# bertoldi-collab/DifFlexMM

Hardware: AMD Instinct MI355X
Metric: timesteps*rigid-units/s (forward + adjoint) (higher is better)
Workload: dtype f64

## Files before the change

difflexmm_amd/csrc/dfx_persist.h:

```cpp
#pragma once
#include "dfx_persist_api.h"

namespace {
using namespace dfx_persist;

typedef unsigned p_u4 __attribute__((ext_vector_type(4)));

__device__ __forceinline__ bool is_poison(double x) { return (unsigned)__double2hiint(x) == kPoisonWord; }

__device__ __forceinline__ void ring_load(const double* place, u32 byte_off, double (&r)[4]) {
  p_u4 c0, c1;
  asm volatile("global_load_dwordx4 %0, %2, %3 sc1\n\tglobal_load_dwordx4 %1, %2, %3 offset:16 sc1\n\ts_waitcnt vmcnt(0)"
               : "=&v"(c0), "=&v"(c1) : "v"(byte_off), "s"(place) : "memory");
  r[0] = __hiloint2double(c0.y, c0.x); r[1] = __hiloint2double(c0.w, c0.z);
  r[2] = __hiloint2double(c1.y, c1.x); r[3] = __hiloint2double(c1.w, c1.z);
}
__device__ __forceinline__ void ring_store(double* place, u32 byte_off, double a, double b) {
  p_u4 x;
  x.x = __double2loint(a); x.y = __double2hiint(a); x.z = __double2loint(b); x.w = __double2hiint(b);
  asm volatile("global_store_dwordx4 %0, %1, %2 sc1\n\ts_nop 1" ::"v"(byte_off), "v"(x), "s"(place) : "memory");
}
__device__ __forceinline__ void ring_poison(double* place, u32 byte_off) {
  p_u4 x; x.x = x.y = x.z = x.w = kPoisonWord;
  asm volatile("global_store_dwordx4 %0, %1, %2 sc1\n\ts_nop 1" ::"v"(byte_off), "v"(x), "s"(place) : "memory");
}

__global__ __launch_bounds__(kThreads) void k_ring_poison(double* ring, int batch, int n_blocks, int m0, int width , int places) {
  const int m = blockIdx.y + m0;
  const int tid = blockIdx.x * kThreads + threadIdx.x;
  if (tid >= n_blocks * width) return;
  const unsigned long long p = ~0ull;
  for (int pl = 0; pl < places; ++pl)
    reinterpret_cast<unsigned long long*>(ring)[((size_t)pl * batch + m) * ((size_t)n_blocks * width) + tid] = p;
}

struct LigRes {
  double rox, roy, rpx, rpy, lx, ly, l0, il0, ks, ksh, kr, sgn;
  double am, ac, kc, phi1, phi2, kap_safe, phi_min;
  int info, pslot;
};
template <int CONTACT, class Ctx >
__device__ __forceinline__ void load_lig_res(const Ctx& c, const MemberBases& B, int slot, LigRes& g) {
  g.info = ldg<int>(c.slot_info, (u32)slot * 4);
  g.pslot = g.info < 0 ? slot : (g.info >> 1);
  g.sgn = (g.info & 1) ? 1.0 : -1.0;
  const double2 ro = ldg<double2>(B.p_r, (u32)slot * 16), rp = ldg<double2>(B.p_r, (u32)g.pslot * 16);
  g.rox = ro.x; g.roy = ro.y; g.rpx = rp.x; g.rpy = rp.y;
  if (c.l_dict_on) {
    const u32 li = (u32)ldg<uint8_t>(B.p_lidx, (u32)slot);
    const double2 lv = ldg<double2>(B.l_dict, li * 32), ln = ldg<double2>(B.l_dict, li * 32 + 16);
    g.lx = lv.x; g.ly = lv.y; g.l0 = ln.x; g.il0 = ln.y;
  } else {
    const double2 lv = ldg<double2>(B.p_l, (u32)slot * 16);
    g.lx = lv.x; g.ly = lv.y;
    g.l0 = g.info < 0 ? 1.0 : sqrt(lv.x * lv.x + lv.y * lv.y);
    g.il0 = 1.0 / g.l0;
  }
  if (c.k_uniform) { g.ks = B.cst[3]; g.ksh = B.cst[4]; g.kr = B.cst[5]; }
  else { g.ks = ldg<double>(B.p_k, (u32)slot * 32); g.ksh = ldg<double>(B.p_k, (u32)slot * 32 + 8); g.kr = ldg<double>(B.p_k, (u32)slot * 32 + 16); }
  g.am = g.ac = g.kc = g.phi1 = g.phi2 = g.kap_safe = g.phi_min = 0.0;
  if (CONTACT == 1) {
    g.am = B.cst[0]; g.ac = B.cst[1]; g.kc = B.cst[2]; g.kap_safe = B.cst[9]; g.phi_min = B.cst[10];
    const double2 ph = ldg<double2>(B.p_phi, (u32)slot * 16);
    g.phi1 = ph.x; g.phi2 = ph.y;
  }
}
__device__ __forceinline__ int fresh_v(int x) { asm volatile("" : "+v"(x)); return x; }
__device__ __forceinline__ MemberBases persist_bases(const PersistCtx& c, u32 um) {
  MemberBases B{};
  const u32 ps = um * (u32)c.n_slots;
  B.p_r = c.p_r + (size_t)(ps * 2); B.p_phi = c.p_phi + (size_t)(ps * 2); B.p_l = c.p_l + (size_t)(ps * 2); B.p_k = c.p_k + (size_t)(ps * 4);
  B.cst = c.cst + (size_t)(um * 16); B.l_dict = c.l_dict + (size_t)(um * 1024); B.p_lidx = c.p_lidx + (size_t)ps;
  return B;
}
__device__ __forceinline__ bool ring_wait(const double* place, u32 byte_off, double (&r)[4], int t_ord, int* give_up, int limit) {
  for (int spins = 0;;) {
    ring_load(place, byte_off, r);
    const bool ok = !(is_poison(r[0]) || is_poison(r[1]) || is_poison(r[2]) || is_poison(r[3]));
    if (__all(ok)) return true;
    if (++spins > limit) { *give_up = 1 + t_ord; return false; }
    __builtin_amdgcn_s_sleep(1);
  }
}

#ifdef DFX_PERSIST_TIMING
__device__ __forceinline__ unsigned long long tick() {
  unsigned long long t;
  asm volatile("s_waitcnt vmcnt(0) lgkmcnt(0)\n\ts_memtime %0\n\ts_waitcnt lgkmcnt(0)" : "=s"(t)::"memory");
  return t;
}
#if DFX_PERSIST_TIMING == 2
#define DFX_TICK(k) if ((k) < 4) { unsigned long long t_; asm volatile("s_memtime %0\n\ts_waitcnt lgkmcnt(0)" : "=s"(t_)::"memory"); acc_t[k] += (unsigned)(t_ - t_prev); t_prev = t_; }
#else
#define DFX_TICK(k) { const unsigned long long t_ = tick(); acc_t[k] += (unsigned)(t_ - t_prev); t_prev = t_; }
#endif
#else
#define DFX_TICK(k)
#endif

__device__ __forceinline__ bool persist_wave(const PersistArgs& pa, int& ml, int& w) {
  const int wv = (int)(threadIdx.x >> 6);
  if (pa.xcd_wg > 0) {
    const int xcd = (int)(blockIdx.x & 7), pos = (int)(blockIdx.x >> 3);
    const int mi = pos / pa.xcd_wg, j = pos - mi * pa.xcd_wg;
    ml = __builtin_amdgcn_readfirstlane(mi * 8 + xcd);
    w = __builtin_amdgcn_readfirstlane(j * (kPersistThreads / 64) + wv);
    return ml < pa.nm && w < pa.waves_per_member;
  }
  const int wave = __builtin_amdgcn_readfirstlane((int)(blockIdx.x * (kPersistThreads / 64)) + wv);
  if (wave >= pa.waves_per_member * pa.nm) return false;
  ml = wave / pa.waves_per_member;
  w = wave - ml * pa.waves_per_member;
  return true;
}

template <int NPB>
__device__ __forceinline__ LanePos wave_lane_pos(int w, int n_blocks) {
  LanePos p;
  const int gtid = w * 64 + (int)(threadIdx.x & 63);
  if (NPB == 4) { p.slot = gtid; p.b = gtid >> 2; p.k = gtid & 3; p.valid = p.b < n_blocks; return p; }
  const int j = gtid & 15;
  const int tri = min((j * 11) >> 5, 4);
  p.k = j - 3 * tri;
  p.b = (gtid >> 4) * 5 + tri;
  p.valid = p.b < n_blocks;
  p.slot = p.b * 4 + p.k;
  return p;
}

#ifndef DFX_PERSIST_OCC
#define DFX_PERSIST_OCC
#endif
template <int MODEL, int CONTACT, int NPB>
__global__ __launch_bounds__(kPersistThreads) DFX_PERSIST_OCC void k_fwd_persist(PersistCtx c, PersistFwdTab pc, PersistArgs pa) {
  int ml, w;
  if (!persist_wave(pa, ml, w)) return;
  const LanePos lp = wave_lane_pos<NPB>(w, c.n_blocks);
  if (!lp.valid) return;
  const int slot = lp.slot, b = lp.b, k = lp.k, kd = k < 3 ? k : 2;
  const u32 um = (u32)ml;
  const u32 nd = (u32)c.n_blocks * 3;
  const int s = c.s;
  const Seg sg = *c.cur;
  const MemberBases B = persist_bases(c, um);
  LigRes g;
  load_lig_res<CONTACT>(c, B, slot, g);
  const int info = g.info, pslot = g.pslot;
  const int dof = b * 3 + kd;
  const u32 o_dof = (u32)dof * 8, o_rec = ((u32)b * kPos + kd) * 8, o_chunk = ((u32)b * kPos + 2 * (k & 1)) * 8;
  const double damp = c.damping_uniform ? B.cst[6 + kd] : ldg<double>(c.damping + (size_t)(um * nd), o_dof);
  const double invm = ldg<double>(c.inv_m + (size_t)(um * nd), o_dof);
  const int sidx = ldg<int>(c.block_special, (u32)b * 4);
  const bool constrained = k < 3 && sidx >= 0 && ((c.special[sidx >= 0 ? sidx : 0].con_mask >> k) & 1);
  double tf_coef[DFX_MAX_FNS];
#pragma unroll
  for (int f = 0; f < DFX_MAX_FNS; ++f)
    tf_coef[f] = (k < 3 && sidx >= 0 && f < c.n_fns) ? (constrained ? c.special[sidx].con_coef[k][f] : c.special[sidx].load_coef[k][f]) : 0.0;
  const bool recs = c.rps > 1;
  const long long n0 = sg.base_step;
  const size_t blk = (size_t)((u32)c.n_blocks * (u32)kStep);
  const size_t rec_step = (size_t)(u32)c.batch * blk;
// ... 2 lines not shown
  double* const VELm = c.VEL + (size_t)(um * (u32)c.nbuf * nd);
  double qn, vn;
  BlockRec<double> o;
  {
    const double* P0 = recs ? traj_m + (size_t)((u32)n0 * (u32)c.rps) * rec_step : POSm;
    const double* V0 = recs ? P0 + (size_t)((u32)c.n_blocks * (u32)kPos) : VELm;
    const double2 a0 = ldg<double2>(P0, (u32)b * kPos * 8), a1 = ldg<double2>(P0, (u32)b * kPos * 8 + 16);
    o.x = a0.x; o.y = a0.y; o.th = a1.x; o.sh = a1.y;
    qn = ldg<double>(P0, o_rec);
    vn = ldg<double>(V0, o_dof);
  }
  double al[kPersistStages];
#pragma unroll
  for (int l = 0; l < kPersistStages; ++l) al[l] = 0.0;
  const size_t ring_stride = (size_t)((u32)c.batch * (u32)c.n_blocks * (u32)kPos);
  const u32 r_own = (um * (u32)c.n_blocks + (u32)b) * (kPos * 8) + 16u * (u32)(k & 1);
  const u32 r_par = (um * (u32)c.n_blocks + (u32)(pslot >> 2)) * (kPos * 8);
  if (k < 2) ring_store(pa.ring, r_own, k == 0 ? o.x : o.th, k == 0 ? o.y : o.sh);
  const int total = pa.n_steps * s;
  int t_ord = 0;
  double v_i = vn;
  const int keep = recs ? 2 : (c.traj ? 1 : 0);
  double* tr = keep ? traj_m + ((size_t)((u32)n0 * (u32)c.rps) + 1) * rec_step : nullptr;
  const size_t rec_adv = recs ? rec_step : 0, rec_gap = recs ? (size_t)(u32)(c.rps - s) * rec_step : (keep ? rec_step : 0);
  const u32 o_vrec = (u32)c.n_blocks * (kPos * 8) + o_dof;
  const double* ft = c.fn_tab ? c.fn_tab + ((size_t)um * kMaxGraphSteps * kFnRows) * (DFX_MAX_FNS * kFnEntry) : nullptr;
  const int ft_row = c.fn_tab ? DFX_MAX_FNS * kFnEntry : 0;
  const u32 z_row = constrained ? (u32)(DFX_MAX_FNS * kFnEntry * 8) : 0u;
  double* Am = c.AD ? c.AD + (size_t)um * c.ad_stride + (size_t)n0 * ((u32)(s - 1) * nd) : nullptr;
  const double* place = pa.ring;
#ifdef DFX_PERSIST_TIMING
  unsigned acc_t[6] = {0, 0, 0, 0, 0, 0};
  unsigned long long t_prev = tick();
  const unsigned long long t_first = t_prev, w_first = wall_clock64();
#endif
  for (int j = 0; j < pa.n_steps; ++j) {
    const long long n = n0 + j;
    double h = sg.h;
    if (c.t_steps) { const double* ts = c.t_steps + (size_t)um * (size_t)c.ts_stride; h = ts[n + 1] - ts[n]; }
#pragma unroll 1
    for (int i = 0; i < s; ++i) {
      {
        const double* row = pc.row[i];
        double cv[kPersistStages - 1], cq[kPersistStages - 1];
#pragma unroll
        for (int l = 0; l < kPersistStages - 1; ++l) { cv[l] = row[l]; cq[l] = row[kPersistStages - 1 + l]; }
        const double cv_i = row[10], cq_i = row[11], c_next = row[12];
        o.ch = half_cos(o.th, o.sh);
        double sv = 0.0, sq = 0.0, fload = 0.0;
#pragma unroll
        for (int l = 0; l < kPersistStages - 1; ++l) {
          sv += cv[l] * al[l];
          sq += cq[l] * al[l];
        }
        double tv0[DFX_MAX_FNS], tv1[DFX_MAX_FNS];
#pragma unroll
        for (int f = 0; f < DFX_MAX_FNS; ++f) { tv0[f] = 0.0; tv1[f] = 0.0; }
        if (k < 3 && sidx >= 0) {
          const u32 z = lane_zero() + z_row;
#pragma unroll
          for (int f = 0; f < DFX_MAX_FNS; ++f)
            if (f < c.n_fns) { tv0[f] = fn_tab_get(ft, f, 0, z); if (constrained) tv1[f] = fn_tab_get(ft, f, 1, z); }
        }
        DFX_TICK(0)
        double pr[4];
        if (!ring_wait(place, r_par, pr, t_ord, pa.give_up, pa.spin_limit)) return;
        DFX_TICK(1)
        if (k < 2 && t_ord + kPAhead <= total) ring_poison(pa.ring + (size_t)(((u32)t_ord + kPAhead) & (kPRing - 1)) * ring_stride, r_own);
        BlockRec<double> p;
        p.x = pr[0]; p.y = pr[1]; p.th = pr[2]; p.sh = pr[3];
        p.ch = half_cos(p.th, p.sh);
        double q_pre = 0.0, v_pre = 0.0;
#pragma unroll
        for (int f = 0; f < DFX_MAX_FNS; ++f) {
          if (constrained) { q_pre += tf_coef[f] * tv0[f]; v_pre += tf_coef[f] * tv1[f]; }
          else fload += tf_coef[f] * tv0[f];
        }
        double fx = 0.0, fy = 0.0, fth = 0.0;
        if (info >= 0) {
          BondGrad<double> bg;
          bond_grad<MODEL, double>(o, p, g.rox, g.roy, g.rpx, g.rpy, g.lx, g.ly, g.l0, g.il0, g.ks, g.ksh, g.kr, g.sgn, bg);
          fx = bg.fx; fy = bg.fy; fth = bg.fth;
          if (CONTACT == 1) {
            const bool far = !(fabs(o.th - p.th) <= g.kap_safe);
            ContactGrad<double> cg;
            contact_grad<double>(g.sgn * (o.th - p.th), far ? g.phi1 : g.phi_min, far ? g.phi2 : g.phi_min, g.am, g.ac, g.kc, cg);
            fth += g.sgn * cg.dkap;
          }
        }
        DFX_TICK(2)
        const double dE = blk_reduce3<NPB>(fx, fy, fth, k);
        double qnext = 0.0, vnext = 0.0;
        if (k < 3) {
          const double a = constrained ? 0.0 : (fload - dE - damp * v_i) * invm;
          if (Am && i < s - 1) stg<double>(Am, o_dof, a);
          sv += cv_i * a;
          sq += cq_i * a;
#pragma unroll
          for (int l = 0; l < kPersistStages; ++l) al[l] = l == i ? a : al[l];
          qnext = qn + h * (c_next * vn + h * sq);
          vnext = vn + h * sv;
          if (constrained) { qnext = q_pre; vnext = v_pre; }
        }
        DFX_TICK(3)
        const double y1 = blk_bcast<NPB, 1>(qnext, k), th2 = blk_bcast<NPB, 2>(qnext, k), x0 = blk_bcast<NPB, 0>(qnext, k);
        double sn, cs;
        fast_sincos(0.5 * th2, &sn, &cs);
        o.x = x0; o.y = y1; o.th = th2; o.sh = sn;
        ++t_ord;
        place = pa.ring + (size_t)((u32)t_ord & (kPRing - 1)) * ring_stride;
        DFX_TICK(4)
        const bool last = i == s - 1;
        if (k < 2) ring_store(const_cast<double*>(place), r_own, k == 0 ? x0 : th2, k == 0 ? y1 : sn);
        if (k < 3) {
          const double2 chunk = k == 0 ? make_double2(x0, y1) : make_double2(th2, sn);
          if (keep > (last ? 0 : 1)) {
            if (k < 2) stg<double2>(tr, o_chunk, chunk);
            stg<double>(tr, o_vrec, vnext);
          }
          if (last && keep < 2 && j == pa.n_steps - 1) {
            if (k < 2) stg<double2>(POSm, o_chunk, chunk);
            stg<double>(VELm, o_dof, vnext);
          }
        }
        v_i = vnext;
        if (last) { qn = qnext; vn = vnext; }
        DFX_TICK(5)
        tr += rec_adv;
        ft += ft_row;
        if (Am && i < s - 1) Am += nd;
      }
    }
    tr += rec_gap;
    ft += (kFnRows - s) * ft_row;
  }
#ifdef DFX_PERSIST_TIMING
  if (pa.dbg && (threadIdx.x & 63) == 0) {
    unsigned* d = pa.dbg + (size_t)(blockIdx.x * 4 + (threadIdx.x >> 6)) * 8;
    for (int q = 0; q < 6; ++q) d[q] = acc_t[q];
    d[6] = (unsigned)(tick() - t_first); d[7] = (unsigned)total;
  }
  if (blockIdx.x == 0 && threadIdx.x == 0) {
    for (int q = 0; q < 6; ++q) pa.give_up[1 + q] = (int)acc_t[q];
    pa.give_up[7] = (int)(tick() - t_first);
    pa.give_up[8] = (int)(wall_clock64() - w_first);
    pa.give_up[9] = total;
  }
#endif
}



template <int MODEL, int CONTACT, int NPB, int DENSE>
__device__ __forceinline__ void adj_persist_body(const PersistCtx& c, const PersistAdjTab& pc, const PersistArgs& pa, const DenseCtx& dn) {
  int ml, w;
  if (!persist_wave(pa, ml, w)) return;
  const LanePos lp = wave_lane_pos<NPB>(w, c.n_blocks);
  if (!lp.valid) return;
  const int slot = lp.slot, b = lp.b, k = lp.k, kd = k < 3 ? k : 2;
  const u32 um = (u32)ml;
  const u32 nd = (u32)c.n_blocks * 3, nd6 = (u32)c.n_blocks * 6;
  const int s = c.s;
  const Seg sg = *c.cur;
  long long n_m = 0;
  int j_top = pa.n_steps - 1;
  if constexpr (DENSE) {
    n_m = dn.n_acc[c.m0 + ml];
    if (n_m - sg.base_step < (long long)j_top) j_top = (int)(n_m - sg.base_step);
    if (j_top < 0) return;
  }
  const MemberBases B = persist_bases(c, um);
  LigRes g;
  load_lig_res<CONTACT>(c, B, slot, g);
  const int info = g.info, pslot = g.pslot;
  const int dof = b * 3 + kd;
  const u32 o_dof = (u32)dof * 8, o_b6 = ((u32)b * 6 + 2 * kd) * 8;
  const double damp = c.damping_uniform ? B.cst[6 + kd] : ldg<double>(c.damping + (size_t)(um * nd), o_dof);
  const double invm = ldg<double>(c.inv_m + (size_t)(um * nd), o_dof);
  const int sidx = ldg<int>(c.block_special, (u32)b * 4);
  const bool constrained = k < 3 && sidx >= 0 && ((c.special[sidx >= 0 ? sidx : 0].con_mask >> k) & 1);
  double tf_coef[DFX_MAX_FNS];
#pragma unroll
  for (int f = 0; f < DFX_MAX_FNS; ++f)
    tf_coef[f] = (k < 3 && sidx >= 0 && f < c.n_fns) ? (constrained ? c.special[sidx].con_coef[k][f] : c.special[sidx].load_coef[k][f]) : 0.0;
  double* LAMm = c.LAM + (size_t)(um * nd6);
  const u32 ms = um * (u32)c.n_slots;
  double* grm = c.g_r + (size_t)(ms * 2);
  double* gpm = c.g_phi + (size_t)ms;
  double* bmm = c.blk_m + (size_t)(um * nd);
  double* bcm = c.blk_c ? c.blk_c + (size_t)(um * nd) : nullptr;
  __shared__ double2 s_yb[kPersistStages - 1][kPersistThreads];
  __shared__ double2 s_racc[kPersistThreads];
  __shared__ double s_acc[3][kPersistThreads];
  __shared__ double2 s_lam[kPersistThreads];
  const int tid = (int)threadIdx.x;
#pragma unroll
  for (int jj = 0; jj < kPersistStages - 1; ++jj) s_yb[jj][tid] = make_double2(0.0, 0.0);
  s_racc[tid] = ldg<double2>(grm, (u32)slot * 16);
  s_lam[tid] = ldg<double2>(LAMm, o_b6);
  s_acc[0][tid] = CONTACT == 1 ? ldg<double>(gpm, (u32)slot * 8) : 0.0;
  s_acc[1][tid] = ldg<double>(bmm, o_dof);
  s_acc[2][tid] = bcm ? ldg<double>(bcm, o_dof) : 0.0;
  bool phi_any = false;
  double* const fn_gq = (c.fn_g && k < 3 && sidx >= 0) ? c.fn_g + (((size_t)um * c.n_special + sidx) * DFX_MAX_FNS) * DFX_FN_PARAMS : nullptr;
  const size_t ring_stride = (size_t)((u32)c.batch * (u32)c.n_blocks * (u32)kPos);
  const u32 r_own = (um * (u32)c.n_blocks + (u32)b) * (kPos * 8) + 16u * (u32)(k & 1);
  const u32 r_par = (um * (u32)c.n_blocks + (u32)(pslot >> 2)) * (kPos * 8);
  const int total = DENSE ? (j_top + 1) * s - ((sg.base_step + j_top == n_m) ? s - 1 : 0) : pa.n_steps * s;
  int t_ord = 0;
  const int i_top = (DENSE && sg.base_step + j_top == n_m) ? 0 : s - 1;
  const size_t rec_step = (size_t)((u32)c.batch * ((u32)c.n_blocks * (u32)kStep));
  const u32 o_vel = (u32)c.n_blocks * (kPos * 8) + o_dof;
  const double* rec = c.traj + (size_t)((((u32)(sg.base_step + j_top) * (u32)c.rps + (u32)i_top) * (u32)c.batch + um)) * (size_t)((u32)c.n_blocks * (u32)kStep);
  const size_t rec_gap = (size_t)(u32)(c.rps - s) * rec_step;
  const double* ft = c.fn_tab ? c.fn_tab + (((size_t)um * kMaxGraphSteps + (u32)j_top) * kFnRows + (u32)i_top) * (DFX_MAX_FNS * kFnEntry) : nullptr;
  const int ft_row = c.fn_tab ? DFX_MAX_FNS * kFnEntry : 0;
  int win = (int)(((sg.base_step + j_top) * s + i_top) & 1);
  const double* place = pa.ring;
#ifdef DFX_PERSIST_TIMING
  unsigned acc_t[6] = {0, 0, 0, 0, 0, 0};
  unsigned long long t_prev = tick();
  const unsigned long long t_first = t_prev;
#endif
  for (int j = j_top; j >= 0; --j) {
    const long long n = sg.base_step + j;
    double h = sg.h, h_before = (sg.j0 + j) == 0 ? sg.h_prev : sg.h;
    if (c.t_steps) { const double* ts = c.t_steps + (size_t)um * (size_t)c.ts_stride; h = ts[n + 1] - ts[n]; h_before = n > 0 ? ts[n] - ts[n - 1] : 0.0; }
    const bool first = !DENSE && (sg.j0 + j) == 0 && c.G;
    double g0q = 0.0, g0v = 0.0;
    if (first && k < 3 && !constrained) {
      const double* G = c.G + ((size_t)sg.interval * c.batch + um) * (size_t)nd6;
      g0q = G[b * 6 + k]; g0v = G[b * 6 + 3 + k];
    }
#pragma unroll 1
    for (int i = (DENSE && n == n_m) ? 0 : s - 1; i >= 0; --i) {
      const double* row = pc.row[i];
      double cf[kPersistStages - 1], cu[kPersistStages - 1];
#pragma unroll
      for (int jj = 0; jj < kPersistStages - 1; ++jj) { cf[jj] = row[jj]; cu[jj] = row[kPersistStages - 1 + jj]; }
// ... 44 lines not shown
          if (i <= 1) {
            double e6q = 0.0, e6v = 0.0, e5v = 0.0;
            for (int kk = plo; kk < lo; ++kk) {
              const double* Gk = c.G + ((size_t)kk * c.batch + um) * (size_t)nd6;
              const double gq = ldg<double>(Gk, o_g), gv = ldg<double>(Gk, o_g + 24);
              const double* wt = dwm + (size_t)kk * 8;
              e6q += wt[6] * gq; e6v += wt[6] * gv;
              e5v += wt[s - 1] * gv;
            }
            if (i == 0) { e_own_q += h_before * e6q; e_own_v += h_before * e6v; e_nxt_v = h_before * e5v; }
            else e_nxt_v += h_before * e6v;
          }
          if (i == 0 && n == 0)
            for (int kk = 0; kk < lo; ++kk) {
              const double* Gk = c.G + ((size_t)kk * c.batch + um) * (size_t)nd6;
              gs_q += ldg<double>(Gk, o_g); gs_v += ldg<double>(Gk, o_g + 24);
            }
          w_d += e_own_v * invm;
        }
      }
      const double wox = blk_bcast<NPB, 0>(w_d, k), woy = blk_bcast<NPB, 1>(w_d, k), woth = blk_bcast<NPB, 2>(w_d, k);
      double wp[4];
      DFX_TICK(0)
      if (t_ord == 0) {
        const double* Win = c.W + (size_t)((um * 2 + (u32)win) * nd);
        const u32 pb = (u32)(pslot >> 2) * 24;
        const double2 wxy = ldg<double2>(Win, pb);
        wp[0] = wxy.x; wp[1] = wxy.y; wp[2] = ldg<double>(Win, pb + 16);
      } else if (!ring_wait(place, r_par, wp, t_ord, pa.give_up, pa.spin_limit)) return;
      DFX_TICK(1)
      if (k < 2 && t_ord + kPAhead < total) ring_poison(pa.ring + (size_t)(((u32)t_ord + kPAhead) & (kPRing - 1)) * ring_stride, r_own);
      BlockRec<double> o, p;
      o.x = o0.x; o.y = o0.y; o.th = o1.x; o.sh = o1.y; o.ch = half_cos(o.th, o.sh);
      p.x = q0.x; p.y = q0.y; p.th = q1.x; p.sh = q1.y; p.ch = half_cos(p.th, p.sh);
      double hx = 0.0, hy = 0.0, hth = 0.0, ex = 0.0, ey = 0.0, eth = 0.0, d_rx = 0.0, d_ry = 0.0, d_phi = 0.0;
      if (info >= 0) {
        BondHvp hv;
        bond_hvp<MODEL>(o, p, wox, woy, woth, wp[0], wp[1], wp[2], g.rox, g.roy, g.rpx, g.rpy, g.lx, g.ly, g.l0, g.il0, g.ks, g.ksh, g.kr, g.sgn, hv);
        hx = hv.hx; hy = hv.hy; hth = hv.hth;
        ex = hv.fx; ey = hv.fy; eth = hv.fth;
        d_rx = hv.rx; d_ry = hv.ry;
        if (CONTACT == 1) {
          const bool far = !(fabs(o.th - p.th) <= g.kap_safe);
          double dk, dke, p1e, p2e;
          contact_hvp(g.sgn * (o.th - p.th), g.sgn * (woth - wp[2]), far ? g.phi1 : g.phi_min, far ? g.phi2 : g.phi_min, g.am, g.ac, g.kc, dk, dke, p1e, p2e);
          hth += g.sgn * dke;
          eth += g.sgn * dk;
          d_phi = (info & 1) ? p2e : p1e;
        }
        const double2 r_old = s_racc[tid];
        s_racc[tid] = make_double2(r_old.x - d_rx, r_old.y - d_ry);
      }
      if (CONTACT == 1 && d_phi != 0.0) { s_acc[0][tid] -= d_phi; phi_any = true; }
      DFX_TICK(2)
      const double hw = blk_reduce3<NPB>(hx, hy, hth, k);
      const double dE = blk_reduce3<NPB>(ex, ey, eth, k);
      double w_next = 0.0;
      if (k < 3) {
        double fload = 0.0;
#pragma unroll
        for (int f = 0; f < DFX_MAX_FNS; ++f) if (!constrained) fload += tf_coef[f] * tv0[f];
        double* const fq = fn_gq;
        if (fresh_v(fq != nullptr)) {
#pragma unroll
          for (int f = 0; f < DFX_MAX_FNS; ++f) {
            const double coef = f < c.n_fns ? (constrained ? -hw * tf_coef[f] : w_d * tf_coef[f]) : 0.0;
            if (coef != 0.0) {
              const u32 z = lane_zero();
              double* q = fq + f * DFX_FN_PARAMS;
              for (int kk = 0; kk < DFX_FN_PARAMS; ++kk) acc_add(q + kk, coef * fn_tab_get(ft, f, 2 + kk, z));
            }
          }
        }
        const double a_i = constrained ? 0.0 : (fload - dE - damp * v_i) * invm;
        double kq_in = h * (cur_s * lq + sqc);
        if constexpr (DENSE) kq_in += e_own_q;
// ... 5 lines not shown
          s_acc[2][tid] -= w_d * v_i;
        }
        if (i > 0) s_yb[i - 1][tid] = make_double2(ybq, ybv);
        double kv;
        if (i > 0) {
          kv = h * (col_s * lv + col_i * ybv + sv);
        } else {
          double nlq = lq + (ybq + sq), nlv = lv + (ybv + sv);
          if constexpr (DENSE) { nlq += gs_q; nlv += gs_v; }
          if (first) { nlq += g0q; nlv += g0v; }
          if (constrained) { nlq = 0.0; nlv = 0.0; }
          s_lam[tid] = make_double2(nlq, nlv);
          kv = h_before * col_s * nlv;
        }
        if constexpr (DENSE) kv += e_nxt_v;
        w_next = constrained ? 0.0 : kv * invm;
      }
      DFX_TICK(3)
      ++t_ord;
      place = pa.ring + (size_t)((u32)t_ord & (kPRing - 1)) * ring_stride;
      if (t_ord < total) {
        const double w1 = blk_bcast<NPB, 1>(w_next, k), w2 = blk_bcast<NPB, 2>(w_next, k);
        if (k < 2) ring_store(const_cast<double*>(place), r_own, k == 0 ? w_next : w2, k == 0 ? w1 : 0.0);
      } else if (k < 3) {
        stg<double>(c.W + (size_t)((um * 2 + (u32)(win ^ 1)) * nd), o_dof, w_next);
      }
      rec -= rec_step;
      ft -= ft_row;
      win ^= 1;
    }
    rec -= rec_gap;
    ft -= (kFnRows - s) * ft_row;
  }
#ifdef DFX_PERSIST_TIMING
  if (pa.dbg && (threadIdx.x & 63) == 0) {
    unsigned* d = pa.dbg + (size_t)(blockIdx.x * 4 + (threadIdx.x >> 6)) * 8;
    for (int q = 0; q < 6; ++q) d[q] = acc_t[q];
    d[6] = (unsigned)(tick() - t_first); d[7] = (unsigned)total;
  }
#endif
  if (info >= 0) stg<double2>(grm, (u32)slot * 16, s_racc[tid]);
  if (CONTACT == 1 && phi_any) { stg<double>(gpm, (u32)slot * 8, s_acc[0][tid]); c.touch[0] = 1; }
  if (k < 3) {
    stg<double2>(LAMm, o_b6, s_lam[tid]);
    if (!constrained) { stg<double>(bmm, o_dof, s_acc[1][tid]); if (bcm) stg<double>(bcm, o_dof, s_acc[2][tid]); }
  }
}

template <int MODEL, int CONTACT, int NPB>
__global__ __launch_bounds__(kPersistThreads) __attribute__((amdgpu_waves_per_eu(3))) void k_adj_persist(PersistCtx c, PersistAdjTab pc, PersistArgs pa) {
  adj_persist_body<MODEL, CONTACT, NPB, 0>(c, pc, pa, DenseCtx{});
}

}
```

difflexmm_amd/csrc/dfx_persist_api.h:

```cpp
#pragma once
#include <hip/hip_runtime.h>

namespace dfx_persist {

constexpr int kPRing = 8;
constexpr int kPAhead = 4;
constexpr int kPersistThreads = 256;
constexpr unsigned kPoisonWord = 0xFFFFFFFFu;
constexpr int kPersistStages = 6;
constexpr int kSpinLimit = 1 << 23;
static_assert(kPAhead >= 2 && kPRing >= kPAhead + 1, "hand-off ring: re-poison at least two ordinals ahead, ring longer than the look-ahead");

struct PersistCoef {
  double cv[kPersistStages][kPersistStages];
  double cq[kPersistStages][kPersistStages];
  double c[kPersistStages + 1];
};
struct PersistArgs {
  double* ring;
  int* give_up;
  int n_steps, nm, waves_per_member;
  int spin_limit;
  int xcd_wg;
#ifdef DFX_PERSIST_TIMING
  unsigned* dbg;
#endif
};


constexpr int kAdjRow = 16;
struct PersistAdjTab { double row[kPersistStages][kAdjRow]; };
struct PersistFwdTab { double row[kPersistStages][kAdjRow]; };
static_assert((kPRing & (kPRing - 1)) == 0, "the ring place of a stage ordinal is taken with a mask");

struct PersistCtx {
  int n_blocks, n_slots, n_fns, batch, s, rps, n_special, m0;
  int k_uniform, damping_uniform, l_dict_on, nbuf;
  const int32_t* slot_info;
  const int32_t* block_special;
  const dfx_special* special;
  const double *p_r, *p_l, *p_k, *p_phi, *l_dict, *cst, *inv_m, *damping;
  const uint8_t* p_lidx;
  const double* fn_tab;
  const dfx::Seg* cur;
  const double* t_steps;
  long long ts_stride;
// ... 17 lines not shown
```

difflexmm_amd/csrc/dfx_persist_dense.h:

```cpp
#pragma once
#include "dfx_persist.h"
#include "dfx_dense.h"

template <int CTRL> __device__ __forceinline__ double dpp_row_mov(double v) {
  int lo = __double2loint(v), hi = __double2hiint(v);
  lo = __builtin_amdgcn_update_dpp(lo, lo, CTRL, 0xf, 0xf, false);
  hi = __builtin_amdgcn_update_dpp(hi, hi, CTRL, 0xf, 0xf, false);
  return __hiloint2double(hi, lo);
}
__device__ __forceinline__ double lanes_plus_32(double v) {
  const unsigned lo = (unsigned)__double2loint(v), hi = (unsigned)__double2hiint(v);
  const auto a = __builtin_amdgcn_permlane32_swap(lo, lo, false, false);
  const auto b = __builtin_amdgcn_permlane32_swap(hi, hi, false, false);
  return __hiloint2double((int)b[1], (int)a[1]);
}
__device__ __forceinline__ double lanes_plus_16(double v) {
  const unsigned lo = (unsigned)__double2loint(v), hi = (unsigned)__double2hiint(v);
  const auto a = __builtin_amdgcn_permlane16_swap(lo, lo, false, false);
  const auto b = __builtin_amdgcn_permlane16_swap(hi, hi, false, false);
  return __hiloint2double((int)b[1], (int)a[1]);
}
__device__ __forceinline__ double wave_sum_lane0(double v) {
  v += lanes_plus_32(v);
  v += lanes_plus_16(v);
// ... 132 lines not shown
#pragma unroll 1
    for (int i = 1; i <= 6; ++i) {
      o.ch = half_cos(o.th, o.sh);
      double sv = 0.0, sq = 0.0, fload = 0.0;
#pragma unroll
      for (int l = 0; l < 6; ++l) {
        const double a_l = l < i ? al[l] : 0.0;
        sv += (i < 6 ? pc.a[i + 1][l] : pc.e[l]) * a_l;
        sq += (i < 6 ? pc.aa[i + 1][l] : pc.ee[l]) * a_l;
      }
      fload = load_at(i);
      double pr[4];
      if (!ring_wait(pa.ring + (size_t)(t_ord % kPRing) * ring_stride, r_par, pr, t_ord, pa.give_up, pa.spin_limit)) return;
      if (valid && k < 2) ring_poison(pa.ring + (size_t)((t_ord + kPAhead) % kPRing) * ring_stride, r_own);
      BlockRec<double> p;
      p.x = pr[0]; p.y = pr[1]; p.th = pr[2]; p.sh = pr[3];
      p.ch = half_cos(p.th, p.sh);
      double fx = 0.0, fy = 0.0, fth = 0.0;
      if (info >= 0) {
        BondGrad<double> bg;
        bond_grad<MODEL, double>(o, p, g.rox, g.roy, g.rpx, g.rpy, g.lx, g.ly, g.l0, g.il0, g.ks, g.ksh, g.kr, g.sgn, bg);
        fx = bg.fx; fy = bg.fy; fth = bg.fth;
        if (CONTACT == 1) {
          const bool far = !(fabs(o.th - p.th) <= g.kap_safe);
          ContactGrad<double> cg;
          contact_grad<double>(g.sgn * (o.th - p.th), far ? g.phi1 : g.phi_min, far ? g.phi2 : g.phi_min, g.am, g.ac, g.kc, cg);
          fth += g.sgn * cg.dkap;
        }
      }
      const double dE = blk_reduce3<4>(fx, fy, fth, k);
      const double a = constrained ? 0.0 : (fload - dE - damp * v_i) * invm;
      ++t_ord;
      if (i < 6) {
        sv += pc.a[i + 1][i] * a;
        sq += pc.aa[i + 1][i] * a;
#pragma unroll
        for (int l = 1; l < 7; ++l) al[l] = l == i ? a : al[l];
        double qx = qn + h * (pc.c[i + 1] * vn + h * sq), vx = vn + h * sv;
        prescribed(i + 1, qx, vx);
        const double y1 = blk_bcast<4, 1>(qx, k), th2 = blk_bcast<4, 2>(qx, k), x0 = blk_bcast<4, 0>(qx, k);
        double sn, cs;
        fast_sincos(0.5 * th2, &sn, &cs);
        o.x = x0; o.y = y1; o.th = th2; o.sh = sn;
        if (valid && k < 2) ring_store(pa.ring + (size_t)(t_ord % kPRing) * ring_stride, r_own, k == 0 ? x0 : th2, k == 0 ? y1 : sn);
        if (keep && dof_lane) {
          double* tr = traj_rec(c, m, -2 - i, n_acc);
          if (k < 2) stg<double2>(tr, o_chunk, k == 0 ? make_double2(x0, y1) : make_double2(th2, sn));
          stg<double>(tr + (size_t)c.n_blocks * kPos, o_dof, vx);
        }
        v_i = vx;
// ... 101 lines not shown
```

difflexmm_amd/csrc/engine_launch.hip:

```cpp
#include "dfx_engine.h"
#include <climits>

using namespace dfx_persist;

void drop_graphs(dfx_handle* h) {
  for (auto& kv : h->graphs) (void)hipGraphExecDestroy(kv.second);
  h->graphs.clear();
  h->graph_ctx_valid = false;
  if (h->adaptive_exec) { (void)hipGraphExecDestroy(h->adaptive_exec); h->adaptive_exec = nullptr; }
}

DevCtx make_ctx(dfx_handle* h) {
  const Plan& pl = h->pl;
  DevCtx c;
  memset(&c, 0, sizeof(c));
  c.n_blocks = pl.n_blocks; c.n_slots = pl.n_slots; c.n_fns = pl.n_fns; c.batch = pl.batch; c.s = pl.tab.s;
#ifdef DFX_ABLATE
  { const char* a = getenv("DFX_ABLATE"); c.ablate = a ? atoi(a) : 0; }
#endif
  c.n_wg = (pl.n_slots + kThreads - 1) / kThreads;
  c.n_wg3 = (pl.n_blocks + (kThreads / 16) * 5 - 1) / ((kThreads / 16) * 5);
  for (int k = 0; k < 4; ++k) c.pred[k] = pl.pred_delta[k];
  c.nbuf = 2 * pl.tab.s;
  c.n_special = pl.n_special; c.k_uniform = h->pp.k_uniform ? 1 : 0; c.n_timepoints = (int)h->ts.size();
// ... 229 lines not shown
    *xcd_wg = 0;
    const char* e = getenv("DFX_PERSIST_XCD");
    const int wg = (int)((wpm + 3) / 4), cus = h->n_cu / 8, per_xcd = (nm + 7) / 8, cap = fn ? persist_cap(fn) : 0;
    if (!(e && e[0] == '0') && h->n_cu % 8 == 0 && wg <= cus && (long long)per_xcd * wg <= (long long)cap * cus) {
      *xcd_wg = wg;
      *grid = 8 * per_xcd * wg;
      *per_cu = std::max(1, (per_xcd * wg + cus - 1) / cus);
      return;
    }
  }
  const long long waves = (long long)nm * wpm;
  const long long g = (waves + 3) / 4;
  *grid = (int)g;
  *per_cu = (int)std::max<long long>(1, (g + h->n_cu - 1) / h->n_cu);
}
static int persist_max_chunks() {
  const char* e = getenv("DFX_PERSIST_CHUNKS");
  return e ? std::max(1, atoi(e)) : 2;
}
static int persist_adj_max_chunks() {
  const char* e = getenv("DFX_PERSIST_ADJ_CHUNKS");
  return e ? std::max(1, atoi(e)) : INT_MAX;
}
static int chunk_members(int nm, int n_chunks, int k) { return nm / n_chunks + (k < nm % n_chunks ? 1 : 0); }
static bool persist_common_ok(dfx_handle* h, const DevCtx& c, bool any_groups = false) {
  if (!persist_shape_ok(h) || h->adaptive || (h->groups.size() != 1 && !any_groups)) return false;
  if (h->pl.n_fns > 0 && !c.fn_tab) return false;
  h->persist_npb = (h->pl.n_npb == 3 && pack3(h)) ? 3 : 4;
  h->persist_wpm = persist_waves_per_member(h, h->persist_npb);
  return true;
}
bool persist_members_ok(const dfx_handle* h, int per_launch) {
  return per_launch > 0 && (h->pl.batch + per_launch - 1) / per_launch <= persist_max_chunks();
}
static bool persist_adj_members_ok(const dfx_handle* h, const void* fn, int per_launch) {
  if (persist_members_ok(h, per_launch)) return true;
  const int nm = h->pl.batch, n_chunks = per_launch > 0 ? (nm + per_launch - 1) / per_launch : 0;
  if (n_chunks <= 0 || n_chunks > persist_adj_max_chunks()) return false;
  const long long room = (long long)persist_cap(fn) * h->n_cu * 4;
  return 2LL * chunk_members(nm, n_chunks, n_chunks - 1) * h->persist_wpm >= room;
}
bool persist_would_serve(dfx_handle* h) {
  if (!persist_shape_ok(h) || h->adaptive || h->groups.size() > 1) return false;
  const int npb = (h->pl.n_npb == 3 && pack3(h)) ? 3 : 4;
  return persist_members_ok(h, persist_members_that_fit(h, dfx_persist::fwd_kernel(h->pl.model, h->pl.contact, npb), npb)) &&
         persist_members_ok(h, persist_members_that_fit(h, dfx_persist::adj_kernel(h->pl.model, h->pl.contact, npb), npb));
// ... 133 lines not shown
  p.blk_m = persist_at(cc.blk_m, m0 * nd); p.blk_c = persist_at(cc.blk_c, m0 * nd);
  p.fn_g = persist_at(cc.fn_g, m0 * (size_t)cc.n_special * DFX_MAX_FNS * DFX_FN_PARAMS);
  p.touch = cc.touch;
  return p;
}
static void launch_segment_persist(dfx_handle* h, const DevCtx& c, hipStream_t st, int nm, int n_steps, bool reverse, double* ring = nullptr) {
  if (!ring) ring = h->d_ring.p;
  const int npb = h->persist_npb, per = reverse ? h->persist_adj_members : h->persist_fwd_members;
  const void* fn = reverse ? dfx_persist::adj_kernel(h->pl.model, h->pl.contact, npb) : dfx_persist::fwd_kernel(h->pl.model, h->pl.contact, npb);
  PersistFwdTab pcf = persist_fwd_tab(h->pl.tab);
  PersistAdjTab pca = persist_adj_tab(h->pl.tab);
  const int n_chunks = (nm + per - 1) / per;
  for (int k = 0, off = 0; k < n_chunks; off += chunk_members(nm, n_chunks, k++)) {
    const int cnt = chunk_members(nm, n_chunks, k);
    DevCtx cc = c;
    cc.m0 = c.m0 + off;
    int grid = 0, per_cu = 0;
    int xcd_wg = 0;
    persist_shape(h, npb, cnt, &grid, &per_cu, fn, &xcd_wg);
    dfx_persist::launch_ring_poison(st, ring, h->pl.batch, h->pl.n_blocks, cc.m0, cnt, kPos);
    h->launches++;
    PersistArgs pa;
    pa.give_up = persist_give_up_word(h); pa.n_steps = n_steps; pa.nm = cnt; pa.waves_per_member = h->persist_wpm; pa.spin_limit = persist_spin_limit(h); pa.xcd_wg = xcd_wg;
#ifdef DFX_PERSIST_TIMING
    pa.dbg = ((reverse ? getenv("DFX_TIMING_REVERSE") != nullptr : getenv("DFX_TIMING_REVERSE") == nullptr) && grid <= 8192) ? persist_dbg_buffer() : nullptr;
#endif
    pa.ring = ring + (size_t)cc.m0 * h->pl.n_blocks * kPos;
    PersistCtx pcx = persist_ctx(cc);
    void* args_f[] = {&pcx, &pcf, &pa};
    void* args_r[] = {&pcx, &pca, &pa};
    launch_persist(h, fn, st, reverse ? args_r : args_f, grid, per_cu * persist_wg_slots(fn));
  }
}
static void launch_fwd_persist(dfx_handle* h, const DevCtx& c, hipStream_t st, int nm, int n_steps) { launch_segment_persist(h, c, st, nm, n_steps, false); }

bool persist_adaptive_plan(dfx_handle* h) {
  h->persist_fwd = false;
  if (!persist_shape_ok(h) || h->groups.size() != 1 || h->pl.tab.s != 6) return false;
  const void* fn = dfx_persist::adaptive_fwd_kernel(h->pl.model, h->pl.contact);
  if (!fn) return false;
  h->persist_npb = 4;
  h->persist_wpm = (h->pl.n_slots + 63) / 64;
  h->persist_fwd_members = persist_members_that_fit(h, fn, 4);
  if (h->persist_fwd_members <= 0 || (h->pl.batch + h->persist_fwd_members - 1) / h->persist_fwd_members > 8) return false;
  const size_t B = h->pl.batch;
  if (h->d_ring.ensure((size_t)kPRing * B * h->pl.n_blocks * kPos) != hipSuccess || h->d_err3.ensure(3 * B * (size_t)h->persist_wpm) != hipSuccess) {
// ... 7 lines not shown
  const void* fn = dfx_persist::adaptive_fwd_kernel(h->pl.model, h->pl.contact);
  const Dopri D = make_dopri();
  AdaptLoopCoef pc;
  memset(&pc, 0, sizeof(pc));
  for (int i = 0; i < 7; ++i) {
    pc.e[i] = D.e[i]; pc.ee[i] = D.ee[i]; pc.cm[i] = D.cm[i]; pc.cma[i] = D.cma[i]; pc.c[i] = D.c[i];
    for (int l = 0; l < 7; ++l) { pc.a[i][l] = D.a[i][l]; pc.aa[i][l] = D.aa[i][l]; }
  }
  const int nm = h->pl.batch, per = h->persist_fwd_members;
  const int n_chunks = (nm + per - 1) / per, even = (nm + n_chunks - 1) / n_chunks;
  aa.err = h->d_err3.p;
  (void)hipMemsetAsync(h->d_err3.p, 0xFF, sizeof(double) * 3 * (size_t)nm * h->persist_wpm, st);
  for (int off = 0; off < nm; off += even) {
    const int cnt = std::min(even, nm - off);
    DevCtx cc = c;
    cc.m0 = c.m0 + off;
    int grid = 0, per_cu = 0;
    int xcd_wg = 0;
    persist_shape(h, 4, cnt, &grid, &per_cu, fn, &xcd_wg);
    dfx_persist::launch_ring_poison(st, h->d_ring.p, h->pl.batch, h->pl.n_blocks, cc.m0, cnt, kPos);
    h->launches++;
    PersistArgs pa;
    pa.ring = h->d_ring.p; pa.give_up = persist_give_up_word(h); pa.n_steps = max_attempts; pa.nm = cnt; pa.waves_per_member = h->persist_wpm; pa.spin_limit = persist_spin_limit(h); pa.xcd_wg = xcd_wg;
#ifdef DFX_PERSIST_TIMING
    pa.dbg = nullptr;
#endif
    void* args[] = {&cc, &pc, &pa, &aa};
    launch_persist(h, fn, st, args, grid, per_cu * persist_wg_slots(fn));
  }
}
bool persist_plan_adj_dense(dfx_handle* h, const DevCtx& c) {
  h->persist_adj = false;
  if (!persist_common_ok(h, c)) return false;
  if (c.rps <= 1 || c.g_b || c.AD || !c.lam_pairs) return false;
  const void* fn = dfx_persist::adj_dense_kernel(h->pl.model, h->pl.contact, h->persist_npb);
  if (!fn) return false;
  h->persist_adj_members = persist_members_that_fit(h, fn, h->persist_npb);
  if (h->persist_adj_members <= 0 || (h->pl.batch + h->persist_adj_members - 1) / h->persist_adj_members > 8) return false;
  if (h->d_ring.ensure((size_t)kPRing * h->pl.batch * h->pl.n_blocks * kPos) != hipSuccess) { (void)hipGetLastError(); return false; }
  h->persist_adj = true;
  return true;
}
void launch_adj_dense_persist(dfx_handle* h, const DevCtx& c, hipStream_t st, int n_steps, DenseCtx dn) {
  const int npb = h->persist_npb, per = h->persist_adj_members, nm = h->pl.batch;
  const void* fn = dfx_persist::adj_dense_kernel(h->pl.model, h->pl.contact, npb);
  PersistAdjTab pca = persist_adj_tab(h->pl.tab);
  const int n_chunks = (nm + per - 1) / per, even = (nm + n_chunks - 1) / n_chunks;
  for (int off = 0; off < nm; off += even) {
    const int cnt = std::min(even, nm - off);
    DevCtx cc = c;
    cc.m0 = c.m0 + off;
    int grid = 0, per_cu = 0;
    int xcd_wg = 0;
    persist_shape(h, npb, cnt, &grid, &per_cu, fn, &xcd_wg);
    dfx_persist::launch_ring_poison(st, h->d_ring.p, h->pl.batch, h->pl.n_blocks, cc.m0, cnt, kPos);
    h->launches++;
    PersistArgs pa;
    pa.ring = h->d_ring.p + (size_t)cc.m0 * h->pl.n_blocks * kPos;
    pa.give_up = persist_give_up_word(h); pa.n_steps = n_steps; pa.nm = cnt; pa.waves_per_member = h->persist_wpm; pa.spin_limit = persist_spin_limit(h); pa.xcd_wg = xcd_wg;
#ifdef DFX_PERSIST_TIMING
    pa.dbg = nullptr;
#endif
    PersistCtx pcx = persist_ctx(cc);
    void* args[] = {&pcx, &pca, &pa, &dn};
    launch_persist(h, fn, st, args, grid, per_cu * persist_wg_slots(fn));
  }
}
static void launch_adj_persist(dfx_handle* h, const DevCtx& c, hipStream_t st, int nm, int n_steps) { launch_segment_persist(h, c, st, nm, n_steps, true); }

static int fin(int i) { return i == 0 ? 0 : 1 + ((i - 1) & 1); }
static int fout(int i, int s) { return i == s - 1 ? 0 : 1 + (i & 1); }
static void launch_fwd_step_stage(dfx_handle* h, const DevCtx& c, hipStream_t st, dim3 grid, int i, int j) {
  const int s = h->pl.tab.s;
  if (c.rps > 1) launch_fwd(h, c, st, grid, i, j, -1 - i, -1 - (i + 1), -1, 0);
  else launch_fwd(h, c, st, grid, i, j, fin(i), fout(i, s), 0, (i == s - 1 && c.traj) ? 1 : 0);
}
static int adj_in_buf(const DevCtx& c, int i) { return c.rps > 1 ? -1 - i : (i == 0 ? -1 : i); }
int step_units(const dfx_handle* h, int kind) { return (kind == 0 ? h->pair_fwd : h->pair_adj) ? h->pl.tab.s / 2 : h->pl.tab.s; }
static void launch_fwd_unit(dfx_handle* h, const DevCtx& c, hipStream_t st, dim3 grid, int u, int j) {
  if (!h->pair_fwd) { launch_fwd_step_stage(h, c, st, grid, u, j); return; }
#ifdef DFX_EXPERIMENTAL
  const int s = h->pl.tab.s, i = 2 * u, nm = (int)grid.y;
// ... 205 lines not shown
```

Measured before the change: 1.365 billion.

## Stagger wave priorities across co-resident persistent members and skip near contact

Gives each co-resident persistent member a distinct hardware wave priority (s_setprio), raising it during compute and dropping it while spinning on the ring. The aim is for members sharing a CU to be served in a staggered order instead of contending evenly. The contact gradient/HVP is now skipped entirely when blocks are within the safe angle, replacing the phi_min evaluation. Pointer advances are also rewritten as byte offsets. The contact change assumes phi_min produced a zero contribution, and the priority scheme adds scalar instructions plus a risk of starving some members.

Result: faster. 1.400 billion (median of 6 runs) (+2.6%).

```diff
diff --git a/difflexmm_amd/csrc/dfx_persist.h b/difflexmm_amd/csrc/dfx_persist.h
--- a/difflexmm_amd/csrc/dfx_persist.h
+++ b/difflexmm_amd/csrc/dfx_persist.h
@@ -36,7 +36,7 @@
 
 struct LigRes {
   double rox, roy, rpx, rpy, lx, ly, l0, il0, ks, ksh, kr, sgn;
-  double am, ac, kc, phi1, phi2, kap_safe, phi_min;
+  double am, ac, kc, phi1, phi2, kap_safe;
   int info, pslot;
 };
 template <int CONTACT, class Ctx >
@@ -58,12 +58,15 @@
   }
   if (c.k_uniform) { g.ks = B.cst[3]; g.ksh = B.cst[4]; g.kr = B.cst[5]; }
   else { g.ks = ldg<double>(B.p_k, (u32)slot * 32); g.ksh = ldg<double>(B.p_k, (u32)slot * 32 + 8); g.kr = ldg<double>(B.p_k, (u32)slot * 32 + 16); }
-  g.am = g.ac = g.kc = g.phi1 = g.phi2 = g.kap_safe = g.phi_min = 0.0;
+  g.am = g.ac = g.kc = g.phi1 = g.phi2 = g.kap_safe = 0.0;
   if (CONTACT == 1) {
-    g.am = B.cst[0]; g.ac = B.cst[1]; g.kc = B.cst[2]; g.kap_safe = B.cst[9]; g.phi_min = B.cst[10];
+    g.am = B.cst[0]; g.ac = B.cst[1]; g.kc = B.cst[2]; g.kap_safe = B.cst[9];
     const double2 ph = ldg<double2>(B.p_phi, (u32)slot * 16);
     g.phi1 = ph.x; g.phi2 = ph.y;
   }
+}
+template <class T> __device__ __forceinline__ T* step_bytes(T* p, long long bytes) {
+  return (T*)((const char*)p + bytes);
 }
 __device__ __forceinline__ int fresh_v(int x) { asm volatile("" : "+v"(x)); return x; }
 __device__ __forceinline__ MemberBases persist_bases(const PersistCtx& c, u32 um) {
@@ -97,6 +100,21 @@
 #else
 #define DFX_TICK(k)
 #endif
+
+__device__ __forceinline__ int prio_rank(const PersistArgs& pa, int ml) {
+  return __builtin_amdgcn_readfirstlane(persist_prio(pa.prio != 0, ml, pa.prio, pa.xcd_wg));
+}
+__device__ __forceinline__ void prio_raise(int& rank) {
+  asm volatile("" : "+s"(rank));
+  if (rank >= 1) {
+    __builtin_amdgcn_s_setprio(1);
+    if (rank >= 2) {
+      __builtin_amdgcn_s_setprio(2);
+      if (rank >= 3) __builtin_amdgcn_s_setprio(3);
+    }
+  }
+}
+__device__ __forceinline__ void prio_drop() { __builtin_amdgcn_s_setprio(0); }
 
 __device__ __forceinline__ bool persist_wave(const PersistArgs& pa, int& ml, int& w) {
   const int wv = (int)(threadIdx.x >> 6);
@@ -137,6 +155,7 @@
   if (!persist_wave(pa, ml, w)) return;
   const LanePos lp = wave_lane_pos<NPB>(w, c.n_blocks);
   if (!lp.valid) return;
+  int rank = prio_rank(pa, ml);
   const int slot = lp.slot, b = lp.b, k = lp.k, kd = k < 3 ? k : 2;
   const u32 um = (u32)ml;
   const u32 nd = (u32)c.n_blocks * 3;
@@ -185,12 +204,13 @@
   double v_i = vn;
   const int keep = recs ? 2 : (c.traj ? 1 : 0);
   double* tr = keep ? traj_m + ((size_t)((u32)n0 * (u32)c.rps) + 1) * rec_step : nullptr;
-  const size_t rec_adv = recs ? rec_step : 0, rec_gap = recs ? (size_t)(u32)(c.rps - s) * rec_step : (keep ? rec_step : 0);
+  const size_t rec_adv = (recs ? rec_step : 0) * 8, rec_gap = (recs ? (size_t)(u32)(c.rps - s) * rec_step : (keep ? rec_step : 0)) * 8;
   const u32 o_vrec = (u32)c.n_blocks * (kPos * 8) + o_dof;
   const double* ft = c.fn_tab ? c.fn_tab + ((size_t)um * kMaxGraphSteps * kFnRows) * (DFX_MAX_FNS * kFnEntry) : nullptr;
-  const int ft_row = c.fn_tab ? DFX_MAX_FNS * kFnEntry : 0;
+  const int ft_row = c.fn_tab ? DFX_MAX_FNS * kFnEntry * 8 : 0;
   const u32 z_row = constrained ? (u32)(DFX_MAX_FNS * kFnEntry * 8) : 0u;
   double* Am = c.AD ? c.AD + (size_t)um * c.ad_stride + (size_t)n0 * ((u32)(s - 1) * nd) : nullptr;
+  const int am_adv = c.AD ? (int)(nd * 8) : 0;
   const double* place = pa.ring;
 #ifdef DFX_PERSIST_TIMING
   unsigned acc_t[6] = {0, 0, 0, 0, 0, 0};
@@ -227,7 +247,9 @@
         }
         DFX_TICK(0)
         double pr[4];
+        prio_drop();
         if (!ring_wait(place, r_par, pr, t_ord, pa.give_up, pa.spin_limit)) return;
+        prio_raise(rank);
         DFX_TICK(1)
         if (k < 2 && t_ord + kPAhead <= total) ring_poison(pa.ring + (size_t)(((u32)t_ord + kPAhead) & (kPRing - 1)) * ring_stride, r_own);
         BlockRec<double> p;
@@ -245,10 +267,11 @@
           bond_grad<MODEL, double>(o, p, g.rox, g.roy, g.rpx, g.rpy, g.lx, g.ly, g.l0, g.il0, g.ks, g.ksh, g.kr, g.sgn, bg);
           fx = bg.fx; fy = bg.fy; fth = bg.fth;
           if (CONTACT == 1) {
-            const bool far = !(fabs(o.th - p.th) <= g.kap_safe);
-            ContactGrad<double> cg;
-            contact_grad<double>(g.sgn * (o.th - p.th), far ? g.phi1 : g.phi_min, far ? g.phi2 : g.phi_min, g.am, g.ac, g.kc, cg);
-            fth += g.sgn * cg.dkap;
+            if (!(fabs(o.th - p.th) <= g.kap_safe)) {
+              ContactGrad<double> cg;
+              contact_grad<double>(g.sgn * (o.th - p.th), g.phi1, g.phi2, g.am, g.ac, g.kc, cg);
+              fth += g.sgn * cg.dkap;
+            }
           }
         }
         DFX_TICK(2)
@@ -275,6 +298,7 @@
         DFX_TICK(4)
         const bool last = i == s - 1;
         if (k < 2) ring_store(const_cast<double*>(place), r_own, k == 0 ? x0 : th2, k == 0 ? y1 : sn);
+        prio_drop();
         if (k < 3) {
           const double2 chunk = k == 0 ? make_double2(x0, y1) : make_double2(th2, sn);
           if (keep > (last ? 0 : 1)) {
@@ -289,13 +313,13 @@
         v_i = vnext;
         if (last) { qn = qnext; vn = vnext; }
         DFX_TICK(5)
-        tr += rec_adv;
-        ft += ft_row;
-        if (Am && i < s - 1) Am += nd;
+        tr = step_bytes(tr, rec_adv);
+        ft = step_bytes(ft, ft_row);
+        Am = step_bytes(Am, i < s - 1 ? am_adv : 0);
       }
     }
-    tr += rec_gap;
-    ft += (kFnRows - s) * ft_row;
+    tr = step_bytes(tr, rec_gap);
+    ft = step_bytes(ft, (kFnRows - s) * ft_row);
   }
 #ifdef DFX_PERSIST_TIMING
   if (pa.dbg && (threadIdx.x & 63) == 0) {
@@ -320,6 +344,7 @@
   if (!persist_wave(pa, ml, w)) return;
   const LanePos lp = wave_lane_pos<NPB>(w, c.n_blocks);
   if (!lp.valid) return;
+  int rank = prio_rank(pa, ml);
   const int slot = lp.slot, b = lp.b, k = lp.k, kd = k < 3 ? k : 2;
   const u32 um = (u32)ml;
   const u32 nd = (u32)c.n_blocks * 3, nd6 = (u32)c.n_blocks * 6;
@@ -364,7 +389,7 @@
   s_acc[0][tid] = CONTACT == 1 ? ldg<double>(gpm, (u32)slot * 8) : 0.0;
   s_acc[1][tid] = ldg<double>(bmm, o_dof);
   s_acc[2][tid] = bcm ? ldg<double>(bcm, o_dof) : 0.0;
-  bool phi_any = false;
+  int phi_any = 0;
   double* const fn_gq = (c.fn_g && k < 3 && sidx >= 0) ? c.fn_g + (((size_t)um * c.n_special + sidx) * DFX_MAX_FNS) * DFX_FN_PARAMS : nullptr;
   const size_t ring_stride = (size_t)((u32)c.batch * (u32)c.n_blocks * (u32)kPos);
   const u32 r_own = (um * (u32)c.n_blocks + (u32)b) * (kPos * 8) + 16u * (u32)(k & 1);
@@ -372,12 +397,12 @@
   const int total = DENSE ? (j_top + 1) * s - ((sg.base_step + j_top == n_m) ? s - 1 : 0) : pa.n_steps * s;
   int t_ord = 0;
   const int i_top = (DENSE && sg.base_step + j_top == n_m) ? 0 : s - 1;
-  const size_t rec_step = (size_t)((u32)c.batch * ((u32)c.n_blocks * (u32)kStep));
+  const size_t rec_step = (size_t)((u32)c.batch * ((u32)c.n_blocks * (u32)kStep)) * 8;
   const u32 o_vel = (u32)c.n_blocks * (kPos * 8) + o_dof;
   const double* rec = c.traj + (size_t)((((u32)(sg.base_step + j_top) * (u32)c.rps + (u32)i_top) * (u32)c.batch + um)) * (size_t)((u32)c.n_blocks * (u32)kStep);
   const size_t rec_gap = (size_t)(u32)(c.rps - s) * rec_step;
   const double* ft = c.fn_tab ? c.fn_tab + (((size_t)um * kMaxGraphSteps + (u32)j_top) * kFnRows + (u32)i_top) * (DFX_MAX_FNS * kFnEntry) : nullptr;
-  const int ft_row = c.fn_tab ? DFX_MAX_FNS * kFnEntry : 0;
+  const int ft_row = c.fn_tab ? DFX_MAX_FNS * kFnEntry * 8 : 0;
   int win = (int)(((sg.base_step + j_top) * s + i_top) & 1);
   const double* place = pa.ring;
 #ifdef DFX_PERSIST_TIMING
@@ -468,18 +493,20 @@
       const double wox = blk_bcast<NPB, 0>(w_d, k), woy = blk_bcast<NPB, 1>(w_d, k), woth = blk_bcast<NPB, 2>(w_d, k);
       double wp[4];
       DFX_TICK(0)
+      prio_drop();
       if (t_ord == 0) {
         const double* Win = c.W + (size_t)((um * 2 + (u32)win) * nd);
         const u32 pb = (u32)(pslot >> 2) * 24;
         const double2 wxy = ldg<double2>(Win, pb);
         wp[0] = wxy.x; wp[1] = wxy.y; wp[2] = ldg<double>(Win, pb + 16);
       } else if (!ring_wait(place, r_par, wp, t_ord, pa.give_up, pa.spin_limit)) return;
+      prio_raise(rank);
       DFX_TICK(1)
       if (k < 2 && t_ord + kPAhead < total) ring_poison(pa.ring + (size_t)(((u32)t_ord + kPAhead) & (kPRing - 1)) * ring_stride, r_own);
       BlockRec<double> o, p;
       o.x = o0.x; o.y = o0.y; o.th = o1.x; o.sh = o1.y; o.ch = half_cos(o.th, o.sh);
       p.x = q0.x; p.y = q0.y; p.th = q1.x; p.sh = q1.y; p.ch = half_cos(p.th, p.sh);
-      double hx = 0.0, hy = 0.0, hth = 0.0, ex = 0.0, ey = 0.0, eth = 0.0, d_rx = 0.0, d_ry = 0.0, d_phi = 0.0;
+      double hx = 0.0, hy = 0.0, hth = 0.0, ex = 0.0, ey = 0.0, eth = 0.0, d_rx = 0.0, d_ry = 0.0;
       if (info >= 0) {
         BondHvp hv;
         bond_hvp<MODEL>(o, p, wox, woy, woth, wp[0], wp[1], wp[2], g.rox, g.roy, g.rpx, g.rpy, g.lx, g.ly, g.l0, g.il0, g.ks, g.ksh, g.kr, g.sgn, hv);
@@ -487,17 +514,18 @@
         ex = hv.fx; ey = hv.fy; eth = hv.fth;
         d_rx = hv.rx; d_ry = hv.ry;
         if (CONTACT == 1) {
-          const bool far = !(fabs(o.th - p.th) <= g.kap_safe);
-          double dk, dke, p1e, p2e;
-          contact_hvp(g.sgn * (o.th - p.th), g.sgn * (woth - wp[2]), far ? g.phi1 : g.phi_min, far ? g.phi2 : g.phi_min, g.am, g.ac, g.kc, dk, dke, p1e, p2e);
-          hth += g.sgn * dke;
-          eth += g.sgn * dk;
-          d_phi = (info & 1) ? p2e : p1e;
+          if (!(fabs(o.th - p.th) <= g.kap_safe)) {
+            double dk, dke, p1e, p2e;
+            contact_hvp(g.sgn * (o.th - p.th), g.sgn * (woth - wp[2]), g.phi1, g.phi2, g.am, g.ac, g.kc, dk, dke, p1e, p2e);
+            hth += g.sgn * dke;
+            eth += g.sgn * dk;
+            const double d_phi = (info & 1) ? p2e : p1e;
+            if (d_phi != 0.0) { s_acc[0][tid] -= d_phi; phi_any = fresh_v(1); }
+          }
         }
         const double2 r_old = s_racc[tid];
         s_racc[tid] = make_double2(r_old.x - d_rx, r_old.y - d_ry);
       }
-      if (CONTACT == 1 && d_phi != 0.0) { s_acc[0][tid] -= d_phi; phi_any = true; }
       DFX_TICK(2)
       const double hw = blk_reduce3<NPB>(hx, hy, hth, k);
       const double dE = blk_reduce3<NPB>(ex, ey, eth, k);
@@ -549,15 +577,16 @@
       if (t_ord < total) {
         const double w1 = blk_bcast<NPB, 1>(w_next, k), w2 = blk_bcast<NPB, 2>(w_next, k);
         if (k < 2) ring_store(const_cast<double*>(place), r_own, k == 0 ? w_next : w2, k == 0 ? w1 : 0.0);
+        prio_drop();
       } else if (k < 3) {
         stg<double>(c.W + (size_t)((um * 2 + (u32)(win ^ 1)) * nd), o_dof, w_next);
       }
-      rec -= rec_step;
-      ft -= ft_row;
+      rec = step_bytes(rec, -(long long)rec_step);
+      ft = step_bytes(ft, -ft_row);
       win ^= 1;
     }
-    rec -= rec_gap;
-    ft -= (kFnRows - s) * ft_row;
+    rec = step_bytes(rec, -(long long)rec_gap);
+    ft = step_bytes(ft, -(kFnRows - s) * ft_row);
   }
 #ifdef DFX_PERSIST_TIMING
   if (pa.dbg && (threadIdx.x & 63) == 0) {
diff --git a/difflexmm_amd/csrc/dfx_persist_api.h b/difflexmm_amd/csrc/dfx_persist_api.h
--- a/difflexmm_amd/csrc/dfx_persist_api.h
+++ b/difflexmm_amd/csrc/dfx_persist_api.h
@@ -1,5 +1,6 @@
 #pragma once
 #include <hip/hip_runtime.h>
+#include "dfx_persist_prio.h"
 
 namespace dfx_persist {
 
@@ -22,6 +23,7 @@
   int n_steps, nm, waves_per_member;
   int spin_limit;
   int xcd_wg;
+  int prio;
 #ifdef DFX_PERSIST_TIMING
   unsigned* dbg;
 #endif
diff --git a/difflexmm_amd/csrc/dfx_persist_dense.h b/difflexmm_amd/csrc/dfx_persist_dense.h
--- a/difflexmm_amd/csrc/dfx_persist_dense.h
+++ b/difflexmm_amd/csrc/dfx_persist_dense.h
@@ -178,10 +178,11 @@
         bond_grad<MODEL, double>(o, p, g.rox, g.roy, g.rpx, g.rpy, g.lx, g.ly, g.l0, g.il0, g.ks, g.ksh, g.kr, g.sgn, bg);
         fx = bg.fx; fy = bg.fy; fth = bg.fth;
         if (CONTACT == 1) {
-          const bool far = !(fabs(o.th - p.th) <= g.kap_safe);
-          ContactGrad<double> cg;
-          contact_grad<double>(g.sgn * (o.th - p.th), far ? g.phi1 : g.phi_min, far ? g.phi2 : g.phi_min, g.am, g.ac, g.kc, cg);
-          fth += g.sgn * cg.dkap;
+          if (!(fabs(o.th - p.th) <= g.kap_safe)) {
+            ContactGrad<double> cg;
+            contact_grad<double>(g.sgn * (o.th - p.th), g.phi1, g.phi2, g.am, g.ac, g.kc, cg);
+            fth += g.sgn * cg.dkap;
+          }
         }
       }
       const double dE = blk_reduce3<4>(fx, fy, fth, k);
diff --git a/difflexmm_amd/csrc/dfx_persist_prio.h b/difflexmm_amd/csrc/dfx_persist_prio.h
--- /dev/null
+++ b/difflexmm_amd/csrc/dfx_persist_prio.h
@@ -0,0 +1,12 @@
+#pragma once
+
+namespace dfx_persist {
+
+constexpr int persist_prio(int mode, int ml, int per_cu, int xcd_wg) {
+  if (mode == 0 || per_cu < 2) return 0;
+  const int ranks = per_cu < 4 ? per_cu : 4;
+  const int r = xcd_wg > 0 ? (ml >> 3) : ml;
+  return 3 - r % ranks;
+}
+
+}
diff --git a/difflexmm_amd/csrc/engine_launch.hip b/difflexmm_amd/csrc/engine_launch.hip
--- a/difflexmm_amd/csrc/engine_launch.hip
+++ b/difflexmm_amd/csrc/engine_launch.hip
@@ -275,6 +275,10 @@
   const char* e = getenv("DFX_PERSIST_ADJ_CHUNKS");
   return e ? std::max(1, atoi(e)) : INT_MAX;
 }
+static bool persist_prio_on() {
+  const char* e = getenv("DFX_PERSIST_PRIO");
+  return !(e && e[0] == '0');
+}
 static int chunk_members(int nm, int n_chunks, int k) { return nm / n_chunks + (k < nm % n_chunks ? 1 : 0); }
 static bool persist_common_ok(dfx_handle* h, const DevCtx& c, bool any_groups = false) {
   if (!persist_shape_ok(h) || h->adaptive || (h->groups.size() != 1 && !any_groups)) return false;
@@ -454,6 +458,7 @@
     h->launches++;
     PersistArgs pa;
     pa.give_up = persist_give_up_word(h); pa.n_steps = n_steps; pa.nm = cnt; pa.waves_per_member = h->persist_wpm; pa.spin_limit = persist_spin_limit(h); pa.xcd_wg = xcd_wg;
+    pa.prio = persist_prio_on() ? per_cu : 0;
 #ifdef DFX_PERSIST_TIMING
     pa.dbg = ((reverse ? getenv("DFX_TIMING_REVERSE") != nullptr : getenv("DFX_TIMING_REVERSE") == nullptr) && grid <= 8192) ? persist_dbg_buffer() : nullptr;
 #endif
@@ -507,6 +512,7 @@
     h->launches++;
     PersistArgs pa;
     pa.ring = h->d_ring.p; pa.give_up = persist_give_up_word(h); pa.n_steps = max_attempts; pa.nm = cnt; pa.waves_per_member = h->persist_wpm; pa.spin_limit = persist_spin_limit(h); pa.xcd_wg = xcd_wg;
+    pa.prio = 0;
 #ifdef DFX_PERSIST_TIMING
     pa.dbg = nullptr;
 #endif
@@ -543,6 +549,7 @@
     PersistArgs pa;
     pa.ring = h->d_ring.p + (size_t)cc.m0 * h->pl.n_blocks * kPos;
     pa.give_up = persist_give_up_word(h); pa.n_steps = n_steps; pa.nm = cnt; pa.waves_per_member = h->persist_wpm; pa.spin_limit = persist_spin_limit(h); pa.xcd_wg = xcd_wg;
+    pa.prio = persist_prio_on() ? per_cu : 0;
 #ifdef DFX_PERSIST_TIMING
     pa.dbg = nullptr;
 #endif
```
